# lutao98/SqrtLM-SLAM

Measured on AMD Instinct MI355X. Metric: LM iterations/sec (synthetic KITTI-00-scale BA), higher is better.
Workload: dtype f64; 1 GPU; synthetic global BA (BASELINE config 4); n_pose=5000, n_landmark=500000, n_obs=4999754, track_len=U{2..18}, robust=False, seed=4, parallelism=landmark-shard x1, comm=none, comm_ranks=1

## Files before the change

sqrtlm-slam_amd/csrc/sqlm_api.cpp:

```cpp
#include <hip/hip_runtime.h>

#include <algorithm>
#include <chrono>
#include <condition_variable>
#include <cstdio>
#include <cmath>
#include <cstring>
#include <functional>
#include <limits>
#include <mutex>
#include <new>
#include <queue>
#include <thread>
#include <sys/mman.h>
#include <unistd.h>
#include <vector>

#include "../../include/sqrtlm.h"
#include "../../include/sqrtlm_orb.h"
#include "se3_dev.h"
#include "sqlm_comm.h"
#include "sqlm_internal.h"

using namespace sqlm;
// ... 101 lines not shown
  bool has_problem = false;
  bool prepared = false;
  bool step_valid = false;
  int n_pose = 0, n_pt = 0;
  int64_t n_obs = 0, n_lid = 0;
  std::vector<double> pose_q, pose_t, intr, pt;
  std::vector<uint8_t> pose_fixed;
  HVec<int32_t> obs_pose, obs_pt;
  HVec<double> obs_uv, obs_info, obs_delta, obs_err;
  HVec<uint8_t> obs_level;
  bool has_stereo = false;
  std::vector<double> obs_ur, pose_bf, obs_err3;
  std::vector<int32_t> lid_pose;
  std::vector<double> lid_pc, lid_pw, lid_n, lid_info, lid_err;
  std::vector<uint8_t> lid_level;
  DevProblem d;
  std::vector<Bucket> buckets;
  std::vector<int> bucket_part_off;
  UpdLaunch upd;
  int n_lm_parts = 0;
  std::vector<int> slot_pt;
  HVec<int64_t> dev_edge;
  std::vector<int64_t> dev_lid_edge;
  std::vector<int> h_btot;
  int max_row_blocks = 0;
  int n_active_edges = 0;
  CRPlan cr;
  int n_cu = 0;
  std::vector<int> cam_pos;
  bool use_tiles = false;
  int tile_max_cp = 0, tile_max_k = 0;
  bool err_pending = false;
  bool err_zero = false;
  bool opt_done = false;
  TilePlan tp;
  TileBuild tb;
  std::vector<std::vector<int>> scat_base;
  std::vector<int> h_kcount, h_span_lo, h_span_hi, h_pt_slot, h_key;
  std::vector<int> h_efirst, h_elast;
  std::vector<uint8_t> h_pose_act, h_pt_act;
  std::vector<DevBuf> bufs;
  std::vector<DevBuf> pins;
  double *h_scalars = nullptr;
  CRSync crs;
  double *mbox = nullptr, *mbox_dev = nullptr;
  unsigned long long mbox_seq = 0;
  bool htrace = false;
  std::chrono::steady_clock::time_point ht_prev{};
  double ht_acc[10] = {};
  int ht_n = 0;
  Comm comm;
  std::vector<int> sh_lo, sh_hi, s_row_host;
  GatherTab gather;
  bool need_maxdiag = false;
  EGSolver *eg = nullptr;
  Sim3Solver *sim3 = nullptr;
  PoseSolver *pose = nullptr;
  LidarSolver *lidar = nullptr;
  OrbEngine *orb = nullptr;
  hipEvent_t ev[2 * SQLM_NKERNEL_TIMERS] = {};
  hipStream_t side = nullptr;
  hipEvent_t ev_fork = nullptr, ev_join = nullptr;
  bool spec = false;
  bool no_pose_fuse = false;
  bool lin_valid = false;
  bool spec_outstanding = false;
// ... 831 lines not shown
    run_threads(nks, [&](int t) {
      int64_t acc = 0;
      for (int s = (int)((int64_t)nL * t / nks); s < (int)((int64_t)nL * (t + 1) / nks); ++s) acc += kcount[pts[s]];
      part[t + 1] = acc;
    });
    for (int t = 0; t < nks; ++t) part[t + 1] += part[t];
    if (part[nks] > (int64_t)std::numeric_limits<int>::max()) return SQLM_ERR_UNSUPPORTED;
    run_threads(nks, [&](int t) {
      int acc = (int)part[t];
      for (int s = (int)((int64_t)nL * t / nks); s < (int)((int64_t)nL * (t + 1) / nks); ++s) {
        acc += kcount[pts[s]];
        lm_begin[s + 1] = acc;
      }
    });
  }
  const int64_t nE = lm_begin[nL];
  if (nE > (int64_t)std::numeric_limits<int>::max()) return SQLM_ERR_UNSUPPORTED;
  phase("  lm_begin");
  c->dev_edge.resize(nE);
  PinVec<int> obs_lm, obs_cam, obs_camh;
  PinVec<double> obs_uv, obs_info, obs_delta, obs_ur;
  PinVec<float> obs_q;
  {
    int e = 0;
    if ((e = pinned(c, P_OBSLM, nE, obs_lm)) || (e = pinned(c, P_OBSCAM, nE, obs_cam)) ||
        (e = pinned(c, P_OBSCAMH, nE, obs_camh)) || (e = pinned(c, P_OBSQ, 4 * nE, obs_q)) ||
        (e = pinned(c, P_OBSUR, c->has_stereo ? nE : 0, obs_ur)))
      return e;
  }
  phase("  pinned");
  const int nth = host_threads(c->n_obs);
  auto par = [&](auto &&fn) { run_threads(nth, fn); };
  std::vector<uint8_t> inexact(nth, 0);
  auto put = [&](int64_t e, int o, int sl, bool &bad) {
    c->dev_edge[o] = e;
    obs_lm[o] = sl;
    obs_cam[o] = c->obs_pose[e];
    obs_camh[o] = phidx[c->obs_pose[e]];
    const double u = c->obs_uv[2 * e], v = c->obs_uv[2 * e + 1], w = c->obs_info[e], dl = c->obs_delta[e];
    const float fu = (float)u, fv = (float)v, fw = (float)w, fd = (float)dl;
    obs_q[4 * (size_t)o] = fu;
    obs_q[4 * (size_t)o + 1] = fv;
    obs_q[4 * (size_t)o + 2] = fw;
    obs_q[4 * (size_t)o + 3] = fd;
    bad |= (double)fu != u || (double)fv != v || (double)fw != w || (double)fd != dl;
    if (c->has_stereo) obs_ur[o] = c->obs_ur[e];
  };
  bool contig = c->n_obs <= (int64_t)std::numeric_limits<int>::max();
  if (contig) {
    std::vector<uint8_t> split(nth, 0);
    par([&](int t) {
      for (int sl = (int)((int64_t)nL * t / nth); sl < (int)((int64_t)nL * (t + 1) / nth); ++sl) {
        const int l = pts[sl];
        if (elast[l] - efirst[l] + 1 != kcount[l]) { split[t] = 1; break; }
      }
    });
    contig = std::find(split.begin(), split.end(), 1) == split.end();
  }
  phase("  contig check");
  if (contig && SQLM_SCATTER_BY_SLOT) {
    par([&](int t) {
      bool bad = false;
      const int s1 = (int)((int64_t)nL * (t + 1) / nth);
      for (int sl = (int)((int64_t)nL * t / nth); sl < s1; ++sl) {
        if (SQLM_SCATTER_PF > 0 && sl + 2 * SQLM_SCATTER_PF < s1) __builtin_prefetch(&efirst[pts[sl + 2 * SQLM_SCATTER_PF]]);
        if (SQLM_SCATTER_PF > 0 && sl + SQLM_SCATTER_PF < s1) {
          const int64_t ep = efirst[pts[sl + SQLM_SCATTER_PF]];
          __builtin_prefetch(&c->obs_uv[2 * ep]);
          __builtin_prefetch(&c->obs_info[ep]);
          __builtin_prefetch(&c->obs_delta[ep]);
          __builtin_prefetch(&c->obs_pose[ep]);
        }
        const int b = lm_begin[sl], k = lm_begin[sl + 1] - b;
        const int64_t e0 = efirst[pts[sl]];
        for (int i = 0; i < k; ++i) put(e0 + i, b + i, sl, bad);
      }
      inexact[t] = bad;
    });
  } else if (contig) {
    par([&](int t) {
      bool bad = false;
      for (int64_t e = c->n_obs * t / nth; e < c->n_obs * (t + 1) / nth; ++e) {
        if (c->obs_level[e] != level) continue;
        const int l = c->obs_pt[e], sl = pt_slot[l];
        put(e, lm_begin[sl] + (int)(e - efirst[l]), sl, bad);
      }
      inexact[t] = bad;
    });
  } else {
    auto ebeg = [&](int t) { return c->n_obs * t / nth; };
    std::vector<std::vector<int>> &base = c->scat_base;
    if ((int)base.size() < nth) base.resize(nth);
    par([&](int t) {
      std::vector<int> &cnt = base[t];
      cnt.assign(nL, 0);
      for (int64_t e = ebeg(t); e < ebeg(t + 1); ++e)
        if (c->obs_level[e] == level) ++cnt[pt_slot[c->obs_pt[e]]];
    });
    par([&](int t) {
      const int s0 = (int)((int64_t)nL * t / nth), s1 = (int)((int64_t)nL * (t + 1) / nth);
      for (int sl = s0; sl < s1; ++sl) {
        int b = lm_begin[sl];
        for (int u = 0; u < nth; ++u) { const int k = base[u][sl]; base[u][sl] = b; b += k; }
      }
    });
    par([&](int t) {
      std::vector<int> &fill = base[t];
      bool bad = false;
      for (int64_t e = ebeg(t); e < ebeg(t + 1); ++e) {
        if (c->obs_level[e] != level) continue;
        const int sl = pt_slot[c->obs_pt[e]];
        put(e, fill[sl]++, sl, bad);
      }
      inexact[t] = bad;
    });
  }
  phase("  scatter");
  const bool obs_f32 = std::find(inexact.begin(), inexact.end(), 1) == inexact.end();
  if (!obs_f32) {
    int e = 0;
    if ((e = pinned(c, P_OBSUV, 2 * nE, obs_uv)) || (e = pinned(c, P_OBSINFO, nE, obs_info)) ||
        (e = pinned(c, P_OBSDELTA, nE, obs_delta)))
      return e;
    par([&](int t) {
      for (int64_t o = nE * t / nth; o < nE * (t + 1) / nth; ++o) {
        const int64_t ed = c->dev_edge[o];
        obs_uv[2 * o] = c->obs_uv[2 * ed];
        obs_uv[2 * o + 1] = c->obs_uv[2 * ed + 1];
        obs_info[o] = c->obs_info[ed];
        obs_delta[o] = c->obs_delta[ed];
      }
    });
  }
  std::vector<int> cam_ptr(nP + 1, 0), cam_obs;
  int64_t n_cam_obs = 0;
  if (sharded) {
    auto obeg = [&](int t) { return nE * t / nth; };
    std::vector<std::vector<int>> base(nth);
    par([&](int t) {
      base[t].assign(nP, 0);
      for (int64_t o = obeg(t); o < obeg(t + 1); ++o)
        if (obs_camh[o] >= 0) ++base[t][obs_camh[o]];
    });
    for (int i = 0; i < nP; ++i)
      for (int u = 0; u < nth; ++u) cam_ptr[i + 1] += base[u][i];
    for (int i = 0; i < nP; ++i) cam_ptr[i + 1] += cam_ptr[i];
    for (int i = 0; i < nP; ++i) {
      int b = cam_ptr[i];
      for (int u = 0; u < nth; ++u) { const int k = base[u][i]; base[u][i] = b; b += k; }
    }
    cam_obs.resize(cam_ptr[nP]);
// ... 300 lines not shown
    const size_t sort_bytes = cam_csr_temp_bytes(nE, nP);
    AL(B_CAMKEY0, (size_t)nE, k0);
    AL(B_CAMKEY1, (size_t)nE, k1);
    AL(B_CAMVAL, (size_t)nE, v0);
    AL(B_SORTTMP, sort_bytes, tmp);
    AL(B_CAMOBS, (size_t)nE, d.cam_obs);
    AL(B_CAMPTR, (size_t)nP + 1, d.cam_obs_ptr);
    if (launch_cam_csr(d.obs_camh, nE, nP, k0, k1, v0, d.cam_obs, d.cam_obs_ptr, tmp, sort_bytes, c->stream))
      return SQLM_ERR_HIP;
  }
  d.has_stereo = c->has_stereo ? 1 : 0;
  if (c->has_stereo) {
    UP(B_POSEBF, c->pose_bf, d.pose_bf);
    AL(B_OBSERR3, (size_t)nE, d.obs_err3);
    AL(B_CAMUR, (size_t)n_cam_obs, d.cam_ur);
  } else {
    d.obs_ur = d.obs_err3 = d.pose_bf = d.cam_ur = nullptr;
  }
  AL(B_CAMSLOT, (size_t)n_cam_obs, d.cam_slot);
  if (d.obs_f32) {
    AL(B_CAMQ, 4 * (size_t)n_cam_obs, d.cam_q);
    d.cam_uv = nullptr;
  } else {
    AL(B_CAMUV, 4 * (size_t)n_cam_obs, d.cam_uv);
    d.cam_q = nullptr;
  }
  launch_cam_gather(d, n_cam_obs, c->stream);
  AL(B_HPP, 36 * (size_t)nP, d.Hpp);
  AL(B_BP, 8 * (size_t)nP, d.bp);
  {
    const bool no_spec = getenv("SQLM_NO_SPEC") && atoi(getenv("SQLM_NO_SPEC")) != 0;
    c->no_pose_fuse = getenv("SQLM_NO_POSE_FUSE") != nullptr;
    c->spec = c->use_tiles && d.obs_P == nullptr && !no_spec;
    c->cam_inline = d.nE < (1 << 18);
    if (sharded) c->cam_inline = false;
  }
  c->lin_valid = false;
  d.pc_lm = kPartChiCurLm;
  d.pc_lid = kPartChiCurLid;
  d.px_lm = kPartChiCurLm2;
  d.px_lid = kPartChiCurLid2;
  if (c->spec) {
    AL(B_LMR_NX, 8 * (size_t)nL, d.lm_R_nx);
    AL(B_LMB_NX, 4 * (size_t)nL, d.lm_b_nx);
    AL(B_OBSS_NX, (size_t)nE, d.obs_s_nx);
    AL(B_HPP_NX, 36 * (size_t)nP, d.Hpp_nx);
    AL(B_BP_NX, 8 * (size_t)nP, d.bp_nx);
  } else {
    d.lm_R_nx = d.lm_b_nx = d.obs_s_nx = d.Hpp_nx = d.bp_nx = nullptr;
  }
  UP(B_LIDPTR, lid_ptr, d.lid_cam_ptr);
  UP(B_LIDDATA, lid_data, d.lid_data);
  UP(B_LIDPOSE, lid_pose, d.lid_pose);
  AL(B_LIDERR, (size_t)d.nLid, d.lid_err);
  UP(B_SROW, s_row, d.s_row_ptr);
  UP(B_SCOL, s_col, d.s_col);
  {
    std::vector<int> srow(s_col.size());
    for (int i = 0; i < nP; ++i)
      for (int k = s_row[i]; k < s_row[i + 1]; ++k) srow[k] = i;
    UP(B_SROWIDX, srow, d.s_row);
  }
  AL(B_S, 36 * (size_t)d.nnzb, d.S);
  AL(B_G, 6 * (size_t)nP, d.g);
  AL(B_DX, 6 * (size_t)nP + 1, d.dx);
  d.cam_pos = nullptr;
  if (c->cr.enabled) {
    const size_t nb = (size_t)c->cr.p * c->cr.n * c->cr.n;
    AL(B_CRD, nb, d.cr_D);
    AL(B_CRL, nb, d.cr_L);
    AL(B_CRE, nb, d.cr_E);
    AL(B_CRA, nb, d.cr_A);
    AL(B_CRC, nb, d.cr_C);
    AL(B_CRG, (size_t)c->cr.p * c->cr.n, d.cr_g);
    AL(B_CRX, (size_t)c->cr.p * c->cr.n, d.cr_x);
    {
      int *dn = nullptr;
      AL(B_CRDONE, (size_t)c->cr.p, dn);
// ... 54 lines not shown
    c->sh_hi.assign(R, 0);
    for (int r = 0; r < R; ++r) { c->sh_lo[r] = rng[2 * r]; c->sh_hi[r] = rng[2 * r + 1]; }
    GatherTab &t = c->gather;
    t.n = 0;
    int64_t off = 0;
    for (int r = 1; r < R; ++r) {
      const int a = c->sh_lo[r], b = c->sh_hi[r];
      t.s_lo[t.n] = 36 * (int64_t)s_row[a];
      t.s_hi[t.n] = 36 * (int64_t)s_row[b];
      t.s_src[t.n] = off;
      off += t.s_hi[t.n] - t.s_lo[t.n];
      t.g_lo[t.n] = 6 * (int64_t)a;
      t.g_hi[t.n] = 6 * (int64_t)b;
      t.g_src[t.n] = off;
      off += t.g_hi[t.n] - t.g_lo[t.n];
      ++t.n;
    }
    if (me == 0) AL(B_XSTAGE, (size_t)std::max<int64_t>(off, 1), d.xstage);
  }
  if (!small.host.empty()) {
    uint8_t *dev = nullptr;
    AL(B_ARENA, small.host.size(), dev);
    PinVec<uint8_t> stg;
    if ((st = pinned(c, P_ARENA, small.host.size(), stg))) return st;
    std::memcpy(stg.data(), small.host.data(), small.host.size());
    SQLM_HIP_OK(hipMemcpyAsync(dev, stg.data(), small.host.size(), hipMemcpyHostToDevice, c->stream));
    for (const auto &[off, p] : small.dst) *p = dev + off;
  }
#undef UP
#undef UPD
#undef AL
  SQLM_HIP_OK(hipMemsetAsync(d.partials, 0, sizeof(double) * kMaxPartials, c->stream));
  SQLM_HIP_OK(hipMemsetAsync(d.maxdiag, 0, sizeof(unsigned long long), c->stream));
  SQLM_HIP_OK(hipMemsetAsync(d.obs_err, 0, sizeof(double) * 2 * std::max<int64_t>(nE, 1), c->stream));
  if (d.obs_err3) SQLM_HIP_OK(hipMemsetAsync(d.obs_err3, 0, sizeof(double) * std::max<int64_t>(nE, 1), c->stream));
  launch_pose_prep(d, 0, c->stream);
  phase("upload");
  if (ptime) {
    (void)hipStreamSynchronize(c->stream);
    phase("gpu drain");
  }
  c->prepared = true;
  return SQLM_OK;
}

void ensure_host_errors(sqlm_ctx *c) {
  if (!c->err_zero) return;
  c->err_zero = false;
  par_assign(c->obs_err, (const double *)nullptr, 2 * (size_t)c->n_obs);
}

int fetch_errors(sqlm_ctx *c) {
  if (!c->err_pending) return SQLM_OK;
  c->err_pending = false;
  if (hipSetDevice(c->device) != hipSuccess) return SQLM_ERR_HIP;
  ensure_host_errors(c);
  DevProblem &d = c->d;
  PinVec<double> err, err3, lerr;
  std::vector<double> fallback[3];
  auto stage = [&](int id, size_t n, PinVec<double> &v, int k) {
    if (pinned(c, id, n, v) == SQLM_OK) return;
    fallback[k].resize(std::max<size_t>(n, 1));
    v.p = fallback[k].data();
    v.n = n;
  };
  stage(P_RERR, 2 * (size_t)d.nE, err, 0);
  stage(P_RERR3, d.obs_err3 ? (size_t)d.nE : 0, err3, 1);
  stage(P_RLERR, (size_t)d.nLid, lerr, 2);
  if (err3.size())
    SQLM_HIP_OK(hipMemcpyAsync(err3.data(), d.obs_err3, err3.size() * sizeof(double), hipMemcpyDeviceToHost, c->stream));
  if (d.nE) SQLM_HIP_OK(hipMemcpyAsync(err.data(), d.obs_err, err.size() * sizeof(double), hipMemcpyDeviceToHost, c->stream));
  if (d.nLid)
    SQLM_HIP_OK(hipMemcpyAsync(lerr.data(), d.lid_err, lerr.size() * sizeof(double), hipMemcpyDeviceToHost, c->stream));
  SQLM_HIP_OK(hipStreamSynchronize(c->stream));
  const int nth = host_threads(d.nE);
  run_threads(nth, [&](int t) {
    for (int64_t o = d.nE * t / nth; o < d.nE * (t + 1) / nth; ++o) {
      c->obs_err[2 * c->dev_edge[o]] = err[2 * o];
      c->obs_err[2 * c->dev_edge[o] + 1] = err[2 * o + 1];
      if (err3.size()) c->obs_err3[c->dev_edge[o]] = err3[o];
    }
  });
  for (int64_t t = 0; t < d.nLid; ++t) c->lid_err[c->dev_lid_edge[t]] = lerr[t];
  return SQLM_OK;
}

int finish(sqlm_ctx *c) {
  DevProblem &d = c->d;
  PinVec<double> qt, X;
  std::vector<double> fallback[2];
  auto stage = [&](int id, size_t n, PinVec<double> &v, int k) {
    if (pinned(c, id, n, v) == SQLM_OK) return;
    fallback[k].resize(std::max<size_t>(n, 1));
    v.p = fallback[k].data();
    v.n = n;
  };
  stage(P_RQT, 8 * (size_t)c->n_pose, qt, 0);
  stage(P_RX, 4 * (size_t)d.nL, X, 1);
  SQLM_HIP_OK(hipMemcpyAsync(qt.data(), d.pose_qt[0], qt.size() * sizeof(double), hipMemcpyDeviceToHost, c->stream));
  if (d.nL) SQLM_HIP_OK(hipMemcpyAsync(X.data(), d.X[0], X.size() * sizeof(double), hipMemcpyDeviceToHost, c->stream));
  SQLM_HIP_OK(hipStreamSynchronize(c->stream));
// ... 2 lines not shown
    for (int k = 0; k < 3; ++k) c->pose_t[3 * p + k] = qt[8 * p + 4 + k];
  }
  const int nth = host_threads(d.nL * 8);
  run_threads(nth, [&](int t) {
    for (int s = (int)((int64_t)d.nL * t / nth); s < (int)((int64_t)d.nL * (t + 1) / nth); ++s)
      for (int k = 0; k < 3; ++k) c->pt[3 * c->slot_pt[s] + k] = X[4 * s + k];
  });
  c->err_pending = d.nE > 0 || d.nLid > 0;
  c->opt_done = true;
  return SQLM_OK;
}

inline void tmark(sqlm_ctx *c, int i, bool end) {
  if (c->timing) (void)hipEventRecord(c->ev[2 * i + (end ? 1 : 0)], c->stream);
}

void acc_events(sqlm_ctx *c, int i0, int i1) {
  if (!c->timing) return;
  for (int i = i0; i < i1; ++i) {
    float ms = 0.f;
    if (hipEventElapsedTime(&ms, c->ev[2 * i], c->ev[2 * i + 1]) == hipSuccess) c->kernel_ms_acc[i] += ms;
  }
}

int linearize(sqlm_ctx *c) {
  DevProblem &d = c->d;
  c->lin_timers = 1;
  if (c->spec && c->lin_valid) {
    tmark(c, 0, false);
    tmark(c, 0, true);
    return SQLM_OK;
  }
  c->lin_timers = 2;
  SQLM_HIP_OK(hipEventRecord(c->ev_fork, c->stream));
  SQLM_HIP_OK(hipStreamWaitEvent(c->side, c->ev_fork, 0));
  if (c->timing) SQLM_HIP_OK(hipEventRecord(c->ev[2], c->side));
  launch_camera_pass(d, c->side);
  if (c->timing) SQLM_HIP_OK(hipEventRecord(c->ev[3], c->side));
  SQLM_HIP_OK(hipEventRecord(c->ev_join, c->side));
  tmark(c, 0, false);
  for (size_t b = 0; b < c->buckets.size(); ++b) launch_linearize(d, c->buckets[b], c->bucket_part_off[b], c->stream);
  tmark(c, 0, true);
  SQLM_HIP_OK(hipStreamWaitEvent(c->stream, c->ev_join, 0));
  if (c->comm.enabled() && c->need_maxdiag) {
    launch_pose_diag(d, c->stream);
    if (comm_allreduce_dev(c->comm, d.hdiag, 6 * (int64_t)d.nP, SQLM_DT_F64, SQLM_OP_SUM, c->stream))
      return SQLM_ERR_COMM;
    launch_pose_maxdiag(d, c->stream);
  }
  return SQLM_OK;
}

struct TrialOut {
  double chi_cur, chi_new, scale, maxdiag;
  bool ok;
  bool dev_err;
};

const double *mbox_wait(sqlm_ctx *c, unsigned long long seq, int &err) {
  err = SQLM_OK;
  const unsigned long long *slot = reinterpret_cast<const unsigned long long *>(c->mbox + kMboxSeq);
  Timer t;
  for (unsigned it = 1;; ++it) {
    if (__atomic_load_n(slot, __ATOMIC_ACQUIRE) == seq) return c->mbox;
    if ((it & 1023) == 0) {
      const hipError_t q = hipStreamQuery(c->stream);
// ... 110 lines not shown
      for (int k = 0; k < t.n; ++k) {
        ops.push_back(P2POp{k + 1, false, d.xstage + t.s_src[k], t.s_hi[k] - t.s_lo[k], SQLM_DT_F64});
        ops.push_back(P2POp{k + 1, false, d.xstage + t.g_src[k], t.g_hi[k] - t.g_lo[k], SQLM_DT_F64});
      }
    } else {
      const int me = c->comm.rank, a = c->sh_lo[me], b = c->sh_hi[me];
      const int64_t s0 = 36 * (int64_t)c->s_row_host[a], s1 = 36 * (int64_t)c->s_row_host[b];
      ops.push_back(P2POp{0, true, d.S + s0, s1 - s0, SQLM_DT_F64});
      ops.push_back(P2POp{0, true, d.g + 6 * (int64_t)a, 6 * (int64_t)(b - a), SQLM_DT_F64});
    }
    if (comm_group_p2p(c->comm, ops, c->stream)) return SQLM_ERR_COMM;
    if (root) launch_gather_add(d, c->gather, c->stream);
  }
  tmark(c, 4, false);
  const bool pose_from_cr = !sharded && c->cr.enabled;
  if (root) {
    s = c->cr.enabled ? launch_cr_solve(d, c->cr, c->stream, !pose_from_cr, &c->crs)
                      : launch_dense_solve(d, c->stream);
    if (s) return s == -2 ? SQLM_ERR_HIP : SQLM_ERR_UNSUPPORTED;
  }
  if (sharded) {
    if (root) launch_flag_pack(d, false, c->stream);
    if (comm_bcast_dev(c->comm, d.dx, 6 * (int64_t)d.nP + 1, SQLM_DT_F64, 0, c->stream)) return SQLM_ERR_COMM;
    if (!root) launch_flag_pack(d, true, c->stream);
  }
  tmark(c, 4, true);
  hmark(c, 3);
  const bool no_fuse = c->no_pose_fuse;
  const bool fuse = pose_from_cr && c->spec && c->cam_inline && !no_fuse && !c->buckets.empty() && !c->buckets[0].wide;
  tmark(c, 5, false);
  if (!fuse) launch_pose_update(d, lambda, c->stream, pose_from_cr);
  tmark(c, 5, true);
  tmark(c, 6, false);
  if (!fuse && c->upd.nb > 0) {
    launch_landmark_update_all(d, c->upd, lambda, c->stream, c->spec);
  } else {
    for (size_t b = 0; b < c->buckets.size(); ++b)
      launch_landmark_update(d, c->buckets[b], lambda, c->bucket_part_off[b], c->stream, c->spec, fuse && b == 0);
  }
  launch_lidar_chi2(d, c->stream);
  tmark(c, 6, true);
  hmark(c, 4);
  cam_after = c->spec && c->cam_inline && !c->timing;
  if (c->spec && !cam_after) return spec_camera_launch(c);
  return SQLM_OK;
}

int trial(sqlm_ctx *c, double lambda, TrialOut &o) {
  bool cam_after = false;
  int s = trial_launch(c, lambda, cam_after);
  if (s) return s;
  tmark(c, 7, false);
  hmark(c, 5);
  s = reduce_and_fetch(c, o, cam_after);
  tmark(c, 7, true);
  hmark(c, 6);
  if (c->htrace) ++c->ht_n;
  acc_events(c, 2, SQLM_NKERNEL_TIMERS);
  return s;
}

void swap_state(sqlm_ctx *c) {
  DevProblem &d = c->d;
  std::swap(d.pose_qt[0], d.pose_qt[1]);
  std::swap(d.pose_rt[0], d.pose_rt[1]);
  std::swap(d.X[0], d.X[1]);
  c->lin_valid = c->spec;
  if (c->spec) {
    std::swap(d.lm_R, d.lm_R_nx);
    std::swap(d.lm_b, d.lm_b_nx);
    std::swap(d.obs_s, d.obs_s_nx);
    std::swap(d.Hpp, d.Hpp_nx);
    std::swap(d.bp, d.bp_nx);
    std::swap(d.pc_lm, d.px_lm);
    std::swap(d.pc_lid, d.px_lid);
  }
}

void flush_cam_timers(sqlm_ctx *c) {
  for (int p = 0; p < 2; ++p) {
    if (!c->cam_pending[p]) continue;
    float ms = 0.f;
    if (hipEventSynchronize(c->ev_cam[p][1]) == hipSuccess &&
        hipEventElapsedTime(&ms, c->ev_cam[p][0], c->ev_cam[p][1]) == hipSuccess)
      c->kernel_ms_acc[1] += ms;
    c->cam_pending[p] = false;
  }
}

int lm_host(sqlm_ctx *c, LMCtl &L, const volatile uint8_t *stop) {
  while (!L.done) {
    if (L.qmax == 0 && L.its > 0) {
      if (stopped(stop)) break;
      c->need_maxdiag = false;
      if (int s = linearize(c)) return s;
    }
    TrialOut o{};
    if (int s = trial(c, L.lambda, o)) return s;
    if (o.dev_err) return SQLM_ERR_HIP;
// ... 968 lines not shown
```

sqrtlm-slam_amd/csrc/sqlm_internal.h:

```cpp
#pragma once
#include <hip/hip_runtime.h>
#include <stdint.h>

#include <cfloat>
#include <cmath>
#include <vector>

#include "../../include/sqrtlm.h"

namespace sqlm {

#define SQLM_HIP_OK(x)                          \
  do {                                          \
    if ((x) != hipSuccess) return SQLM_ERR_HIP; \
  } while (0)

#ifndef SQLM_TILE_MAXCAMS
#define SQLM_TILE_MAXCAMS 24
#endif
#ifndef SQLM_TILE_MAXLM
#define SQLM_TILE_MAXLM 128
#endif
constexpr int kTileMaxCams = SQLM_TILE_MAXCAMS, kTileHardCams = 24, kTileMaxLm = SQLM_TILE_MAXLM, kTileMaxK = 1 << 20;
constexpr int kTileNtMax = (6 * kTileHardCams + 15) / 16;
// ... 56 lines not shown
    c.its++;
    c.qmax = 0;
    c.done = c.its >= c.iterations || stop || (c.result != 0 && !c.bench);
  }
  return acc;
}

struct DevProblem {
  int n_pose = 0, nP = 0, nL = 0;
  int sharded = 0, rank = 0;
  int64_t nE = 0;
  double *pose_qt[2] = {nullptr, nullptr};
  double *pose_rt[2] = {nullptr, nullptr};
  double *intr = nullptr;
  int *pose_hidx = nullptr;
  int *hidx_pose = nullptr;
  double *X[2] = {nullptr, nullptr};
  int *lm_begin = nullptr;
  double *lm_R = nullptr;
  double *lm_b = nullptr;
  double *lm_R_nx = nullptr, *lm_b_nx = nullptr, *obs_s_nx = nullptr, *Hpp_nx = nullptr, *bp_nx = nullptr;
  double *lm_M = nullptr;
  double *lm_v = nullptr;
  int *obs_lm = nullptr;
  int *obs_cam = nullptr;
  int *obs_camh = nullptr;
  double *obs_uv = nullptr;
  double *obs_info = nullptr;
  double *obs_delta = nullptr;
  int obs_f32 = 0;
  float *obs_q = nullptr;
  float *cam_q = nullptr;
  double *obs_s = nullptr;
  double *obs_P = nullptr;
  double *obs_err = nullptr;
  int has_stereo = 0;
  double *obs_ur = nullptr;
  double *obs_err3 = nullptr;
  double *pose_bf = nullptr;
  double *cam_ur = nullptr;
  int *cam_obs_ptr = nullptr;
  int *cam_obs = nullptr;
  int *cam_slot = nullptr;
  double *cam_uv = nullptr;
  double *Hpp = nullptr;
  double *bp = nullptr;
  int64_t nLid = 0;
  int *lid_cam_ptr = nullptr;
  double *lid_data = nullptr;
  int *lid_pose = nullptr;
  double *lid_err = nullptr;
  int64_t nnzb = 0;
  int *s_row_ptr = nullptr;
  int *s_col = nullptr;
  int *s_row = nullptr;
  double *S = nullptr;
  double *g = nullptr;
  double *dx = nullptr;
  double *hdiag = nullptr;
  double *xstage = nullptr;
  int dense_n = 0;
  double *dense = nullptr;
  double *dense_L = nullptr;
  double *dense_Linv = nullptr;
  double *dense_r = nullptr, *dense_x = nullptr;
  int n_tiles = 0;
  int *tile_order = nullptr;
  int tile_cls_off[kTileNtMax + 2] = {}, tile_cls_cnt[kTileNtMax + 1] = {};
// ... 63 lines not shown
  std::vector<int> sched;
  const int *sched_dev = nullptr;
  std::vector<int> lvl;
  int init_off = 0, init_cnt = 0;
  int elim_off = 0, elim_cnt = 0;
  bool top_active = false;
};
constexpr int kCRMaxN = 112;
constexpr int kBandMaxCams = kCRMaxN / 6 - 1;
constexpr int kUpdHad = 1 << 28, kUpdRight = 1 << 29, kUpdLeft = 1 << 30, kUpdMask = (1 << 28) - 1;

__host__ __device__ inline int tile_blk(int u, int w, int cp) { return u * (2 * cp - u + 1) / 2 + (w - u); }

#ifndef SQLM_OBS_PER_LANE
#define SQLM_OBS_PER_LANE 3
#endif
constexpr int kObsPerLane = SQLM_OBS_PER_LANE;
#ifndef SQLM_OBS_PRELOAD
#define SQLM_OBS_PRELOAD 2
#endif
constexpr int kObsPreload = SQLM_OBS_PRELOAD;

constexpr int kUpdWin = 64;
struct Bucket {
  int W;
  int slot_begin;
  int slot_end;
  int rng_off = 0;
  bool wide = false;
};

void launch_pose_prep(const DevProblem &d, int buf, hipStream_t st);
void launch_linearize(const DevProblem &d, const Bucket &b, int part_off, hipStream_t st);
void launch_camera_pass(const DevProblem &d, hipStream_t st, bool spec = false);
void launch_pose_maxdiag(const DevProblem &d, hipStream_t st);
void launch_pose_diag(const DevProblem &d, hipStream_t st);
void launch_cam_gather(const DevProblem &d, int64_t n_cam_obs, hipStream_t st);
size_t cam_csr_temp_bytes(int64_t n, int nP);
int launch_cam_csr(const int *camh, int64_t n, int nP, unsigned *keys_in, unsigned *keys_out, int *vals_in,
                   int *cam_obs, int *cam_ptr, void *temp, size_t temp_bytes, hipStream_t st);
constexpr int kMaxRanks = 16;
struct GatherTab {
  int n = 0;
  int64_t s_lo[kMaxRanks], s_hi[kMaxRanks], s_src[kMaxRanks];
  int64_t g_lo[kMaxRanks], g_hi[kMaxRanks], g_src[kMaxRanks];
};
void launch_gather_add(const DevProblem &d, const GatherTab &t, hipStream_t st);
void launch_flag_pack(const DevProblem &d, bool unpack, hipStream_t st);
void launch_damp(const DevProblem &d, double lambda, hipStream_t st);
void launch_rcs(const DevProblem &d, double lambda, int max_row_blocks, hipStream_t st);
struct TileStreams {
  hipStream_t s[2] = {nullptr, nullptr};
  hipEvent_t fork = nullptr, join[2] = {nullptr, nullptr};
};
void launch_rcs_tiles(const DevProblem &d, double lambda, int max_cp, int max_k, hipStream_t st,
                      const TileStreams *ts = nullptr);
int rcs_tile_kernel(const DevProblem &d);
void launch_rcs_reduce(const DevProblem &d, double lambda, hipStream_t st);
#ifdef SQLM_TILE_PROF
int tile_profile_read(long long *out);
#endif
constexpr int kRedLong = 24;
int launch_dense_solve(const DevProblem &d, hipStream_t st);
struct CRSync {
  int *done = nullptr;
  int cap = 0, epoch = 0;
// ... 216 lines not shown
```

sqrtlm-slam_amd/csrc/sqlm_kernels.hip:

```cpp
#include <hip/hip_runtime.h>

#include <type_traits>

#include <algorithm>

#include <cstring>
#ifdef SQLM_TILE_HTRACE
#include <chrono>
#include <cstdio>
#endif
#include <rocprim/device/device_radix_sort.hpp>

#include "se3_dev.h"
#include "sqlm_internal.h"

namespace sqlm {


__device__ __forceinline__ double wave_sum(double v) {
#pragma unroll
  for (int off = 32; off >= 1; off >>= 1) v += __shfl_xor(v, off, 64);
  return v;
}

// ... 218 lines not shown


__global__ void k_pose_prep(const double *__restrict__ qt, const double *__restrict__ intr,
                            double *__restrict__ rt, int n) {
  const int p = blockIdx.x * blockDim.x + threadIdx.x;
  if (p >= n) return;
  double q[4] = {qt[8 * p], qt[8 * p + 1], qt[8 * p + 2], qt[8 * p + 3]};
  double R[9];
  q_to_mat(q, R);
  double *o = rt + 16 * p;
#pragma unroll
  for (int i = 0; i < 9; ++i) o[i] = R[i];
  o[9] = qt[8 * p + 4]; o[10] = qt[8 * p + 5]; o[11] = qt[8 * p + 6];
  o[12] = intr[4 * p]; o[13] = intr[4 * p + 1]; o[14] = intr[4 * p + 2]; o[15] = intr[4 * p + 3];
}

void launch_pose_prep(const DevProblem &d, int buf, hipStream_t st) {
  if (d.n_pose == 0) return;
  hipLaunchKernelGGL(k_pose_prep, dim3((d.n_pose + 255) / 256), dim3(256), 0, st, d.pose_qt[buf], d.intr,
                     d.pose_rt[buf], d.n_pose);
}

template <bool ST>
__device__ __forceinline__ void lin_edge(const DevProblem &d, const ObsIn &o, int e, const double *prt_all, double X0,
                                         double X1, double X2, double *s_out, bool want_P, double R[6], double &b0,
                                         double &b1, double &b2, double &g0, double &g1, double &g2, double &chi) {
  const int cam = o.cam;
  const double *prt = prt_all + 16 * cam;
  MonoEval m;
  const double bf = ST ? d.pose_bf[cam] : 0.0;
  const bool st = ST && o.ur >= 0.0;
  if (st) stereo_error(prt, X0, X1, X2, o.u, o.v, o.ur, bf, o.info, o.delta, m);
  else mono_error(prt, X0, X1, X2, o.u, o.v, o.info, o.delta, m);
  store2(d.obs_err + 2 * e, m.e0, m.e1);
  if (ST) d.obs_err3[e] = st ? m.e2 : 0.0;
  s_out[e] = m.s;
  chi += m.chi_rob;
  double jl[6], jp[12], jl3[3] = {0, 0, 0}, jp3[6] = {0, 0, 0, 0, 0, 0};
  mono_jac(prt, m, jl, jp);
  const double r0 = m.s * m.e0, r1 = m.s * m.e1;
  b0 -= jl[0] * r0 + jl[3] * r1;
  b1 -= jl[1] * r0 + jl[4] * r1;
  b2 -= jl[2] * r0 + jl[5] * r1;
  g0 += jl[0] * jl[0] + jl[3] * jl[3];
  g1 += jl[1] * jl[1] + jl[4] * jl[4];
  g2 += jl[2] * jl[2] + jl[5] * jl[5];
  givens_add_row(R, jl[0], jl[1], jl[2]);
  givens_add_row(R, jl[3], jl[4], jl[5]);
  if (st) {
    stereo_row(prt, m, bf, jl, jp, jl3, jp3);
    const double r2 = m.s * m.e2;
    b0 -= jl3[0] * r2; b1 -= jl3[1] * r2; b2 -= jl3[2] * r2;
    g0 += jl3[0] * jl3[0]; g1 += jl3[1] * jl3[1]; g2 += jl3[2] * jl3[2];
    givens_add_row(R, jl3[0], jl3[1], jl3[2]);
  }
  if (want_P && d.obs_P && o.camh >= 0) {
    double *P = d.obs_P + e;
#pragma unroll
    for (int a = 0; a < 3; ++a)
#pragma unroll
      for (int c = 0; c < 6; ++c)
        P[(6 * a + c) * d.nE] = jl[a] * jp[c] + jl[3 + a] * jp[6 + c] + (st ? jl3[a] * jp3[c] : 0.0);
  }
}

template <int OFF>
__device__ __forceinline__ double seg_xor(double v) {
  if constexpr (OFF <= 8) {
    constexpr int ctrl = OFF == 1 ? 0xB1 : OFF == 2 ? 0x4E : OFF == 4 ? 0x141 : 0x140;
// ... 80 lines not shown
      double *Ro = d.lm_R + 8 * slot;
      store2(Ro, R[0], R[1]); store2(Ro + 2, R[2], R[3]); store2(Ro + 4, R[4], R[5]);
      double *bo = d.lm_b + 4 * slot;
      store2(bo, b0, b1); store2(bo + 2, b2, 0.0);
      chi_acc += chi;
      dmax = fmax(dmax, fmax(g0, fmax(g1, g2)));
    }
  }
  const double s = block_sum(chi_acc, red);
  const double mx = block_max(dmax, red);
  if (threadIdx.x == 0) {
    d.partials[d.pc_lm + part_off + blockIdx.x] = s;
    atomicMax(d.maxdiag, (unsigned long long)__double_as_longlong(mx));
  }
}

void launch_linearize(const DevProblem &d, const Bucket &b, int part_off, hipStream_t st) {
  const int nb = linearize_blocks(b);
  if (nb <= 0) return;
  switch (b.W) {
#define SQLM_CASE(WW)                                                                                          \
  case WW:                                                                                                     \
    if (d.has_stereo)                                                                                          \
      hipLaunchKernelGGL((k_linearize<WW, true>), dim3(nb), dim3(kBlock), 0, st, d, b.slot_begin, b.slot_end,  \
                         part_off);                                                                            \
    else                                                                                                       \
      hipLaunchKernelGGL((k_linearize<WW, false>), dim3(nb), dim3(kBlock), 0, st, d, b.slot_begin, b.slot_end, \
                         part_off);                                                                            \
    break;
    SQLM_CASE(2) SQLM_CASE(4) SQLM_CASE(8) SQLM_CASE(16) SQLM_CASE(32) SQLM_CASE(64)
#undef SQLM_CASE
    default: break;
  }
}


#ifndef SQLM_CAM_OCC
#define SQLM_CAM_OCC 5
#endif
template <bool ST, bool LID>
__global__ __launch_bounds__(256, LID ? 1 : SQLM_CAM_OCC) void k_camera_pass(DevProblem d, int spec) {
  const int wave = threadIdx.x >> 6, lane = threadIdx.x & 63;
  const double *pose_rt_s = spec ? d.pose_rt[1] : d.pose_rt[0], *X_s = spec ? d.X[1] : d.X[0];
  const double *pose_qt_s = spec ? d.pose_qt[1] : d.pose_qt[0];
  const int i = __builtin_amdgcn_readfirstlane(blockIdx.x * 4 + wave);
  double H[21], b[6], chi = 0.0;
#pragma unroll
  for (int k = 0; k < 21; ++k) H[k] = 0.0;
#pragma unroll
  for (int k = 0; k < 6; ++k) b[k] = 0.0;
  if (i < d.nP) {
    const double *prt = pose_rt_s + 16 * d.hidx_pose[i];
    const double bf = ST ? d.pose_bf[d.hidx_pose[i]] : 0.0;
    for (int t = d.cam_obs_ptr[i] + lane; t < d.cam_obs_ptr[i + 1]; t += 64) {
      const double *X = X_s + 4 * d.cam_slot[t];
      double2 uv, id;
      if (d.obs_f32) {
        const float4 q = *reinterpret_cast<const float4 *>(d.cam_q + 4 * (int64_t)t);
        uv = make_double2(q.x, q.y);
        id = make_double2(q.z, q.w);
      } else {
        uv = *reinterpret_cast<const double2 *>(d.cam_uv + 4 * t);
        id = *reinterpret_cast<const double2 *>(d.cam_uv + 4 * t + 2);
      }
      const double ur = ST ? d.cam_ur[t] : -1.0;
      const bool st = ST && ur >= 0.0;
// ... 1421 lines not shown
      oi.v = q.y;
      oi.info = q.z;
      oi.delta = q.w;
      return oi;
    };
    auto stream2 = [&](auto &&use) {
      int e = beg + lane + kObsPreload * W;
      if (park) {
#pragma unroll 1
        for (int j = 0; j < kUpdCache && e < end; ++j, e += W) use(parked(j), e);
      }
      for (; e < end; e += W) use(load_obs<ST, true>(d, e, true), e);
    };
    a0 = seg_sum<W>(a0); a1 = seg_sum<W>(a1); a2 = seg_sum<W>(a2);
    double chi = 0.0;
    double R[6] = {0, 0, 0, 0, 0, 0};
    double b0 = 0, b1 = 0, b2 = 0, g0 = 0, g1 = 0, g2 = 0;
    if (valid) {
      const double *bl = d.lm_b + 4 * slot;
      double Ri[6], wl[3];
      damp_factor(d.lm_R + 8 * slot, bl, lambda, Ri, wl);
      const double c0 = bl[0] - a0, c1 = bl[1] - a1, c2 = bl[2] - a2;
      const double y0 = Ri[0] * c0, y1 = Ri[1] * c0 + Ri[3] * c1, y2 = Ri[2] * c0 + Ri[4] * c1 + Ri[5] * c2;
      const double dl0 = Ri[0] * y0 + Ri[1] * y1 + Ri[2] * y2;
      const double dl1 = Ri[3] * y1 + Ri[4] * y2;
      const double dl2 = Ri[5] * y2;
      const double X0 = L0 + dl0, X1 = L1 + dl1, X2 = L2 + dl2;
      if (lane == 0) {
        double *Xo = d.X[1] + 4 * slot;
        store2(Xo, X0, X1); store2(Xo + 2, X2, 0.0);
        sc_acc += dl0 * (lambda * dl0 + bl[0]) + dl1 * (lambda * dl1 + bl[1]) + dl2 * (lambda * dl2 + bl[2]);
      }
      if (SPEC) {
#pragma unroll
        for (int i = 0; i < kObsPreload; ++i) {
          const int e = beg + lane + i * W;
          if (e < end) lin_edge<ST>(d, o[i], e, P1, X0, X1, X2, d.obs_s_nx, false, R, b0, b1, b2, g0, g1, g2, chi);
        }
        stream2([&](const ObsIn &oi, int e) {
          lin_edge<ST>(d, oi, e, P1, X0, X1, X2, d.obs_s_nx, false, R, b0, b1, b2, g0, g1, g2, chi);
        });
      } else {
        auto trial_err = [&](const ObsIn &o, int e) {
          MonoEval m;
          const double *prt = P1 + 16 * o.cam;
          if (ST && o.ur >= 0.0) stereo_error(prt, X0, X1, X2, o.u, o.v, o.ur, d.pose_bf[o.cam], o.info, o.delta, m);
          else mono_error(prt, X0, X1, X2, o.u, o.v, o.info, o.delta, m);
          store2(d.obs_err + 2 * e, m.e0, m.e1);
          if (ST) d.obs_err3[e] = o.ur >= 0.0 ? m.e2 : 0.0;
          chi += m.chi_rob;
        };
#pragma unroll
        for (int i = 0; i < kObsPreload; ++i)
          if (beg + lane + i * W < end) trial_err(o[i], beg + lane + i * W);
        stream2([&](const ObsIn &oi, int e) { trial_err(oi, e); });
      }
    }
    if (SPEC) {
      lin_butterfly<W>(lane, R, b0, b1, b2, g0, g1, g2, chi);
      if (valid && lane == 0) {
        double *Ro = d.lm_R_nx + 8 * slot;
        store2(Ro, R[0], R[1]); store2(Ro + 2, R[2], R[3]); store2(Ro + 4, R[4], R[5]);
        double *bo = d.lm_b_nx + 4 * slot;
        store2(bo, b0, b1); store2(bo + 2, b2, 0.0);
      }
    } else {
      chi = seg_sum<W>(chi);
    }
    if (valid && lane == 0) chi_acc += chi;
  };
  for (int tile = bid; tile < ntiles; tile += nlm_blocks) {
    const int2 rg = rng[tile];
    TileIn tin;
    if constexpr (!FUSE) tin = tile_load(tile);
    const int nw = rg.y - rg.x + 1;
    if (nw <= kUpdWin) {
      lds_barrier();
      if constexpr (FUSE) {
        for (int k = threadIdx.x; k < 16 * nw; k += blockDim.x) Wp0[k] = d.pose_rt[0][16 * rg.x + k];
        for (int c = threadIdx.x; c < nw; c += blockDim.x) {
          const int p = rg.x + c;
          double q[4], t3[3], dd[6], R[9];
// ... 237 lines not shown
```

Baseline: 581.9 LM iterations/s.

## Defer per-edge residual stores to result readback and skip robust-weight writes

Removes the per-edge residual stores (obs_err/obs_err3) from the speculative linearize and trial-error kernels in the hot LM loop. When results are read back, a new k_edge_errors kernel recomputes them from a tracked buffer state. When no observation uses a robust kernel (all delta <= 0), the per-edge robust-weight array is treated as constant: the next-iteration buffer aliases the current one and its writes are skipped. This saves several doubles of global write traffic per edge per iteration, at the cost of an extra error pass at readback and extra state to keep consistent across buffer swaps.

```diff
diff --git a/sqrtlm-slam_amd/csrc/sqlm_api.cpp b/sqrtlm-slam_amd/csrc/sqlm_api.cpp
--- a/sqrtlm-slam_amd/csrc/sqlm_api.cpp
+++ b/sqrtlm-slam_amd/csrc/sqlm_api.cpp
@@ -157,6 +157,8 @@
   int tile_max_cp = 0, tile_max_k = 0;
   bool err_pending = false;
   bool err_zero = false;
+  int err_state = -1;
+  bool trial_stores = false;
   bool opt_done = false;
   TilePlan tp;
   TileBuild tb;
@@ -1054,7 +1056,7 @@
   const int nth = host_threads(c->n_obs);
   auto par = [&](auto &&fn) { run_threads(nth, fn); };
   std::vector<uint8_t> inexact(nth, 0);
-  auto put = [&](int64_t e, int o, int sl, bool &bad) {
+  auto put = [&](int64_t e, int o, int sl, uint8_t &flg) {
     c->dev_edge[o] = e;
     obs_lm[o] = sl;
     obs_cam[o] = c->obs_pose[e];
@@ -1065,7 +1067,8 @@
     obs_q[4 * (size_t)o + 1] = fv;
     obs_q[4 * (size_t)o + 2] = fw;
     obs_q[4 * (size_t)o + 3] = fd;
-    bad |= (double)fu != u || (double)fv != v || (double)fw != w || (double)fd != dl;
+    flg |= ((double)fu != u || (double)fv != v || (double)fw != w || (double)fd != dl) ? 1 : 0;
+    flg |= dl > 0.0 ? 2 : 0;
     if (c->has_stereo) obs_ur[o] = c->obs_ur[e];
   };
   bool contig = c->n_obs <= (int64_t)std::numeric_limits<int>::max();
@@ -1082,7 +1085,7 @@
   phase("  contig check");
   if (contig && SQLM_SCATTER_BY_SLOT) {
     par([&](int t) {
-      bool bad = false;
+      uint8_t bad = 0;
       const int s1 = (int)((int64_t)nL * (t + 1) / nth);
       for (int sl = (int)((int64_t)nL * t / nth); sl < s1; ++sl) {
         if (SQLM_SCATTER_PF > 0 && sl + 2 * SQLM_SCATTER_PF < s1) __builtin_prefetch(&efirst[pts[sl + 2 * SQLM_SCATTER_PF]]);
@@ -1101,7 +1104,7 @@
     });
   } else if (contig) {
     par([&](int t) {
-      bool bad = false;
+      uint8_t bad = 0;
       for (int64_t e = c->n_obs * t / nth; e < c->n_obs * (t + 1) / nth; ++e) {
         if (c->obs_level[e] != level) continue;
         const int l = c->obs_pt[e], sl = pt_slot[l];
@@ -1128,7 +1131,7 @@
     });
     par([&](int t) {
       std::vector<int> &fill = base[t];
-      bool bad = false;
+      uint8_t bad = 0;
       for (int64_t e = ebeg(t); e < ebeg(t + 1); ++e) {
         if (c->obs_level[e] != level) continue;
         const int sl = pt_slot[c->obs_pt[e]];
@@ -1138,7 +1141,9 @@
     });
   }
   phase("  scatter");
-  const bool obs_f32 = std::find(inexact.begin(), inexact.end(), 1) == inexact.end();
+  uint8_t obs_flg = 0;
+  for (uint8_t f : inexact) obs_flg |= f;
+  const bool obs_f32 = (obs_flg & 1) == 0, any_robust = (obs_flg & 2) != 0;
   if (!obs_f32) {
     int e = 0;
     if ((e = pinned(c, P_OBSUV, 2 * nE, obs_uv)) || (e = pinned(c, P_OBSINFO, nE, obs_info)) ||
@@ -1505,6 +1510,9 @@
     const bool no_spec = getenv("SQLM_NO_SPEC") && atoi(getenv("SQLM_NO_SPEC")) != 0;
     c->no_pose_fuse = getenv("SQLM_NO_POSE_FUSE") != nullptr;
     c->spec = c->use_tiles && d.obs_P == nullptr && !no_spec;
+    c->trial_stores = getenv("SQLM_TRIAL_STORES") && atoi(getenv("SQLM_TRIAL_STORES")) != 0;
+    d.trial_stores = c->trial_stores ? 1 : 0;
+    d.s_const = !any_robust && !c->trial_stores ? 1 : 0;
     c->cam_inline = d.nE < (1 << 18);
     if (sharded) c->cam_inline = false;
   }
@@ -1516,7 +1524,8 @@
   if (c->spec) {
     AL(B_LMR_NX, 8 * (size_t)nL, d.lm_R_nx);
     AL(B_LMB_NX, 4 * (size_t)nL, d.lm_b_nx);
-    AL(B_OBSS_NX, (size_t)nE, d.obs_s_nx);
+    if (d.s_const) d.obs_s_nx = d.obs_s;
+    else AL(B_OBSS_NX, (size_t)nE, d.obs_s_nx);
     AL(B_HPP_NX, 36 * (size_t)nP, d.Hpp_nx);
     AL(B_BP_NX, 8 * (size_t)nP, d.bp_nx);
   } else {
@@ -1637,8 +1646,7 @@
 #undef AL
   SQLM_HIP_OK(hipMemsetAsync(d.partials, 0, sizeof(double) * kMaxPartials, c->stream));
   SQLM_HIP_OK(hipMemsetAsync(d.maxdiag, 0, sizeof(unsigned long long), c->stream));
-  SQLM_HIP_OK(hipMemsetAsync(d.obs_err, 0, sizeof(double) * 2 * std::max<int64_t>(nE, 1), c->stream));
-  if (d.obs_err3) SQLM_HIP_OK(hipMemsetAsync(d.obs_err3, 0, sizeof(double) * std::max<int64_t>(nE, 1), c->stream));
+  c->err_state = -1;
   launch_pose_prep(d, 0, c->stream);
   phase("upload");
   if (ptime) {
@@ -1672,6 +1680,12 @@
   stage(P_RERR, 2 * (size_t)d.nE, err, 0);
   stage(P_RERR3, d.obs_err3 ? (size_t)d.nE : 0, err3, 1);
   stage(P_RLERR, (size_t)d.nLid, lerr, 2);
+  if (c->err_state < 0) {
+    if (d.nE) SQLM_HIP_OK(hipMemsetAsync(d.obs_err, 0, sizeof(double) * 2 * (size_t)d.nE, c->stream));
+    if (d.nE && d.obs_err3) SQLM_HIP_OK(hipMemsetAsync(d.obs_err3, 0, sizeof(double) * (size_t)d.nE, c->stream));
+  } else if (!c->trial_stores) {
+    launch_edge_errors(d, c->err_state, c->stream);
+  }
   if (err3.size())
     SQLM_HIP_OK(hipMemcpyAsync(err3.data(), d.obs_err3, err3.size() * sizeof(double), hipMemcpyDeviceToHost, c->stream));
   if (d.nE) SQLM_HIP_OK(hipMemcpyAsync(err.data(), d.obs_err, err.size() * sizeof(double), hipMemcpyDeviceToHost, c->stream));
@@ -1740,6 +1754,7 @@
     return SQLM_OK;
   }
   c->lin_timers = 2;
+  c->err_state = 0;
   SQLM_HIP_OK(hipEventRecord(c->ev_fork, c->stream));
   SQLM_HIP_OK(hipStreamWaitEvent(c->side, c->ev_fork, 0));
   if (c->timing) SQLM_HIP_OK(hipEventRecord(c->ev[2], c->side));
@@ -1916,6 +1931,7 @@
   if (!fuse) launch_pose_update(d, lambda, c->stream, pose_from_cr);
   tmark(c, 5, true);
   tmark(c, 6, false);
+  c->err_state = 1;
   if (!fuse && c->upd.nb > 0) {
     launch_landmark_update_all(d, c->upd, lambda, c->stream, c->spec);
   } else {
@@ -1949,6 +1965,7 @@
   std::swap(d.pose_qt[0], d.pose_qt[1]);
   std::swap(d.pose_rt[0], d.pose_rt[1]);
   std::swap(d.X[0], d.X[1]);
+  if (c->err_state >= 0) c->err_state ^= 1;
   c->lin_valid = c->spec;
   if (c->spec) {
     std::swap(d.lm_R, d.lm_R_nx);
diff --git a/sqrtlm-slam_amd/csrc/sqlm_internal.h b/sqrtlm-slam_amd/csrc/sqlm_internal.h
--- a/sqrtlm-slam_amd/csrc/sqlm_internal.h
+++ b/sqrtlm-slam_amd/csrc/sqlm_internal.h
@@ -112,8 +112,10 @@
   float *obs_q = nullptr;
   float *cam_q = nullptr;
   double *obs_s = nullptr;
+  int s_const = 0;
   double *obs_P = nullptr;
   double *obs_err = nullptr;
+  int trial_stores = 0;
   int has_stereo = 0;
   double *obs_ur = nullptr;
   double *obs_err3 = nullptr;
@@ -243,6 +245,7 @@
 
 void launch_pose_prep(const DevProblem &d, int buf, hipStream_t st);
 void launch_linearize(const DevProblem &d, const Bucket &b, int part_off, hipStream_t st);
+void launch_edge_errors(const DevProblem &d, int buf, hipStream_t st);
 void launch_camera_pass(const DevProblem &d, hipStream_t st, bool spec = false);
 void launch_pose_maxdiag(const DevProblem &d, hipStream_t st);
 void launch_pose_diag(const DevProblem &d, hipStream_t st);
diff --git a/sqrtlm-slam_amd/csrc/sqlm_kernels.hip b/sqrtlm-slam_amd/csrc/sqlm_kernels.hip
--- a/sqrtlm-slam_amd/csrc/sqlm_kernels.hip
+++ b/sqrtlm-slam_amd/csrc/sqlm_kernels.hip
@@ -274,9 +274,11 @@
   const bool st = ST && o.ur >= 0.0;
   if (st) stereo_error(prt, X0, X1, X2, o.u, o.v, o.ur, bf, o.info, o.delta, m);
   else mono_error(prt, X0, X1, X2, o.u, o.v, o.info, o.delta, m);
-  store2(d.obs_err + 2 * e, m.e0, m.e1);
-  if (ST) d.obs_err3[e] = st ? m.e2 : 0.0;
-  s_out[e] = m.s;
+  if (d.trial_stores) {
+    store2(d.obs_err + 2 * e, m.e0, m.e1);
+    if (ST) d.obs_err3[e] = st ? m.e2 : 0.0;
+  }
+  if (s_out) s_out[e] = m.s;
   chi += m.chi_rob;
   double jl[6], jp[12], jl3[3] = {0, 0, 0}, jp3[6] = {0, 0, 0, 0, 0, 0};
   mono_jac(prt, m, jl, jp);
@@ -423,6 +425,30 @@
 #undef SQLM_CASE
     default: break;
   }
+}
+
+
+template <bool ST>
+__global__ __launch_bounds__(256) void k_edge_errors(DevProblem d, int buf) {
+  const int64_t t = (int64_t)blockIdx.x * blockDim.x + threadIdx.x;
+  if (t >= d.nE) return;
+  const int e = (int)t;
+  const ObsIn o = load_obs<ST, false>(d, e, true);
+  const double *X = d.X[buf] + 4 * (int64_t)d.obs_lm[e];
+  const double *prt = d.pose_rt[buf] + 16 * o.cam;
+  const bool st = ST && o.ur >= 0.0;
+  MonoEval m;
+  if (st) stereo_error(prt, X[0], X[1], X[2], o.u, o.v, o.ur, d.pose_bf[o.cam], o.info, o.delta, m);
+  else mono_error(prt, X[0], X[1], X[2], o.u, o.v, o.info, o.delta, m);
+  store2(d.obs_err + 2 * t, m.e0, m.e1);
+  if (ST) d.obs_err3[e] = st ? m.e2 : 0.0;
+}
+
+void launch_edge_errors(const DevProblem &d, int buf, hipStream_t st) {
+  if (d.nE <= 0) return;
+  const dim3 grid((unsigned)((d.nE + 255) / 256));
+  if (d.has_stereo) hipLaunchKernelGGL(k_edge_errors<true>, grid, dim3(256), 0, st, d, buf);
+  else hipLaunchKernelGGL(k_edge_errors<false>, grid, dim3(256), 0, st, d, buf);
 }
 
 
@@ -1910,13 +1936,14 @@
         sc_acc += dl0 * (lambda * dl0 + bl[0]) + dl1 * (lambda * dl1 + bl[1]) + dl2 * (lambda * dl2 + bl[2]);
       }
       if (SPEC) {
+        double *s_nx = d.s_const ? nullptr : d.obs_s_nx;
 #pragma unroll
         for (int i = 0; i < kObsPreload; ++i) {
           const int e = beg + lane + i * W;
-          if (e < end) lin_edge<ST>(d, o[i], e, P1, X0, X1, X2, d.obs_s_nx, false, R, b0, b1, b2, g0, g1, g2, chi);
+          if (e < end) lin_edge<ST>(d, o[i], e, P1, X0, X1, X2, s_nx, false, R, b0, b1, b2, g0, g1, g2, chi);
         }
         stream2([&](const ObsIn &oi, int e) {
-          lin_edge<ST>(d, oi, e, P1, X0, X1, X2, d.obs_s_nx, false, R, b0, b1, b2, g0, g1, g2, chi);
+          lin_edge<ST>(d, oi, e, P1, X0, X1, X2, s_nx, false, R, b0, b1, b2, g0, g1, g2, chi);
         });
       } else {
         auto trial_err = [&](const ObsIn &o, int e) {
@@ -1924,8 +1951,10 @@
           const double *prt = P1 + 16 * o.cam;
           if (ST && o.ur >= 0.0) stereo_error(prt, X0, X1, X2, o.u, o.v, o.ur, d.pose_bf[o.cam], o.info, o.delta, m);
           else mono_error(prt, X0, X1, X2, o.u, o.v, o.info, o.delta, m);
-          store2(d.obs_err + 2 * e, m.e0, m.e1);
-          if (ST) d.obs_err3[e] = o.ur >= 0.0 ? m.e2 : 0.0;
+          if (d.trial_stores) {
+            store2(d.obs_err + 2 * e, m.e0, m.e1);
+            if (ST) d.obs_err3[e] = o.ur >= 0.0 ? m.e2 : 0.0;
+          }
           chi += m.chi_rob;
         };
 #pragma unroll
```

Result: faster. 593.0 LM iterations/s, median of 6 (+1.9%).
